# MiloszKrajewski/K4os.Compression.LZ4

Hardware: AMD Instinct MI355X
Metric: GiB/s encode+decode on batched 64 KiB blocks; bit-exact vs C# ref (higher is better)
Workload: dtype u8

## Files before the change

experiments/parse_cost_order/fit.py:

```python
import ctypes as C, os, sys, subprocess, numpy as np
ROOT = os.path.dirname(os.path.dirname(os.path.dirname(os.path.abspath(__file__))))
sys.path.insert(0, ROOT)
WORK = sys.argv[1]
from k4os.compression.lz4_amd import corpus
so = os.path.join(WORK, "libstudy.so")
lib = C.CDLL(so)
n, bs = 4096, 65536
cache = os.path.join(WORK, "blocks.npy")
if os.path.exists(cache): blocks = np.load(cache)
else:
    blocks = corpus.silesia_like_blocks(n, bs, seed=2); np.save(cache, blocks)
uidx = np.array([ci + 12 * t for ci in range(12) for t in range(32)])
ub = np.ascontiguousarray(blocks[uidx])
off = (np.arange(384, dtype=np.uint64) * bs); lens = np.full(384, bs, np.int32)
def stats(o, l):
    out = np.zeros((384, 8), np.uint32)
    lib.study_stats(ub.ctypes.data_as(C.POINTER(C.c_uint8)), C.c_void_p(off.ctypes.data), C.c_void_p(lens.ctypes.data), C.c_longlong(384), C.c_uint32(o), C.c_uint32(l), C.c_void_p(out.ctypes.data), C.c_int(8), C.c_uint32(0))
    return out[:, :6].astype(np.float64), out[:, 6].astype(np.float64)
b = np.arange(n); u = (b % 12) * 32 + (b // 12) % 32
ls = np.zeros(384); ln = np.zeros(384); ms = np.zeros(384); mn = np.zeros(384)
for f in ("parent_blocks", "oracleP_blocks", "oracleQ_blocks"):
    res = np.load(os.path.join(WORK, "%s.npy" % f))
    for r in res:
        d = (r[:, 1] - r[:, 0]) / 1e5; k = r[:, 2].astype(int)
        np.add.at(ls, u[k == 4], d[k == 4]); np.add.at(ln, u[k == 4], 1)
        np.add.at(ms, u[k != 4], d[k != 4]); np.add.at(mn, u[k != 4], 1)
lds = np.where(ln > 0, ls / np.maximum(ln, 1), np.nan); mem = np.where(mn > 0, ms / np.maximum(mn, 1), np.nan)
both = (ln >= 2) & (mn >= 2)
ratio = np.median(mem[both] / lds[both]); print("ratio", ratio, "both", both.sum(), "lds known", (ln > 0).sum())
truth = np.where(np.isnan(lds), mem / ratio, lds)
np.save(os.path.join(WORK, "truth.npy"), truth)
names = corpus.SILESIA_NAMES
def evaluate(tag, est):
    e = est[u] + 1e-9 * np.random.default_rng(0).random(n)
    t = truth[u]
    cut = np.sort(e)[::-1][2303]
    inl = e >= cut
    tail_mem = (t[~inl] * ratio).max(); tail_lds = t[inl].max()
    tcut = np.sort(t)[::-1][2303]
    mis = ((t >= tcut) & ~inl).sum()
# ... 28 lines not shown
```

experiments/parse_cost_order/fit_stats.cpp:

```cpp
#include "hip/hip_runtime.h"
#include "k4lz4_decode.hpp"
#include "k4lz4_encode_fast.hpp"
#include "k4lz4_parse.hpp"
#include <vector>

namespace k4 {
__global__ void stats_kernel(BatchArgs a, uint32_t off, uint32_t len, uint32_t *out, uint32_t cap = 0)
{
    __shared__ __attribute__((aligned(16))) uint32_t lds[PCOST_WAVES_PER_WG][4096 + PARSE_SEEN_DWORDS];
    const int lane = lane_id();
    const uint32_t wave = uni(threadIdx.x >> 6);
    const long long b = (long long)blockIdx.x * PCOST_WAVES_PER_WG + (long long)wave;
    if (b >= a.n) return;
    const uint32_t src_len = (uint32_t)a.srcLen[b];
    uint32_t o = off, s = len;
    if (o + s > src_len) { o = 0; s = s < src_len ? s : src_len; }
    ParseStats st; st.max_rounds = cap;
    const uint32_t nseq = parse_block<1, false, true>(a.src + a.srcOff[b] + o, s, nullptr, (uint16_t *)lds[wave], lds[wave] + 4096, lane, nullptr, &st);
    if (lane == 0) { uint32_t *w = out + 8 * b; w[0] = st.rounds; w[1] = st.slow; w[2] = nseq; w[3] = st.groups; w[4] = st.lazies; w[5] = st.longs; w[6] = st.covered; }
}
}

extern "C" int study_stats(const uint8_t *src, const uint64_t *srcOff, const int32_t *srcLen, long long n, uint32_t off, uint32_t len, uint32_t *out, int threads, uint32_t cap)
{
    k4::BatchArgs a{};
    a.src = src; a.srcOff = srcOff; a.srcLen = srcLen; a.n = n; a.accel = 1;
    k4emu::launch_fn(dim3((unsigned)((n + k4::PCOST_WAVES_PER_WG - 1) / k4::PCOST_WAVES_PER_WG)), dim3(64 * k4::PCOST_WAVES_PER_WG), [=] { k4::stats_kernel(a, off, len, out, cap); }, threads);
    return 0;
}
```

k4os/compression/lz4_amd/csrc/k4lz4_capi.hip:

```cpp
#include <hip/hip_runtime.h>
#include <stdint.h>
#include <stdio.h>
#include <stdlib.h>
#include <string.h>
#include <algorithm>
#include <atomic>
#include <memory>
#include <new>
#include <condition_variable>
#include <functional>
#include <map>
#include <mutex>
#include <string>
#include <thread>
#include <chrono>
#include <vector>

#include "../../../../include/k4lz4.h"
#include "k4lz4_decode.hpp"
#include "k4lz4_encode_fast.hpp"
#include "k4lz4_parse.hpp"
#include "k4lz4_pickle.hpp"
#include "k4lz4_segments.hpp"
#include "k4lz4_encode_hc.hpp"
// ... 554 lines not shown
            a.seg_first = sg.first; a.seg_items = sg.items; a.seg_snaps = sg.snaps;
            seg = true;
        }
        auto segments_start = [&]() -> int {
            if (!seg) return K4LZ4_OK;
            K4_HIP(ctx, hipEventRecord(ctx->ev_fork, stream));
            K4_HIP(ctx, hipStreamWaitEvent(ctx->aux2, ctx->ev_fork, 0));
            hipLaunchKernelGGL(k4::k4_encode_seg_kernel, dim3((unsigned)((sg.max_items + k4::ENCODE_WAVES_PER_WG - 1) / k4::ENCODE_WAVES_PER_WG)), dim3(64 * k4::ENCODE_WAVES_PER_WG), 0, ctx->aux2, a, sg);
            K4_HIP(ctx, hipEventRecord(ctx->ev_join2, ctx->aux2));
            return K4LZ4_OK;
        };
        auto segments_join = [&]() -> int {
            if (!seg) return K4LZ4_OK;
            K4_HIP(ctx, hipStreamWaitEvent(stream, ctx->ev_join2, 0));
            hipLaunchKernelGGL(k4::k4_seg_join_kernel, dim3((unsigned)std::min<int64_t>(k4::SEG_MAX_BLOCKS, cnt)), dim3(64), 0, stream, a, sg);
            return K4LZ4_OK;
        };
        if (dd && dd->dict) {
            a.dict = dd->dict; a.dictOff = dd->off + first; a.dictLen = dd->len + first;
            a.dictMode = dd->mode ? dd->mode + first : nullptr;
        }
        if (reorder && parse_path && kind == KIND_ENCODE && ctx->parse_pcost) {
            const int64_t wgs = std::min<int64_t>((cnt + k4::PARSE_MAX_WAVES - 1) / k4::PARSE_MAX_WAVES, ctx->cu_count);
            const size_t need = (size_t)wgs * (k4::PARSE_MAX_WAVES - k4::PARSE_LDS_TABLES) * 16384;
            if (need > ctx->d_parse_cap) K4_HIP(ctx, hipStreamSynchronize(stream));
            const int rcp = grow(ctx, &ctx->d_parse, &ctx->d_parse_cap, need, false);
            if (rcp != K4LZ4_OK) return rcp;
            a.cost = d_cost; a.hist = d_hist; a.order_out = d_order;
            K4_HIP(ctx, hipMemsetAsync(d_hist, 0, 2 * k4::PCOST_BUCKETS * 4, stream));
            k4::ParseCost pc = ctx->pcost_fit;
            pc.tables = (uint32_t *)ctx->d_parse;
            hipLaunchKernelGGL(static_cast<void (*)(k4::BatchArgs, k4::ParseCost)>(k4::k4_cost_kernel), dim3((unsigned)wgs), dim3(64 * k4::PARSE_MAX_WAVES), 0, stream, a, pc);
            hipLaunchKernelGGL(k4::k4_order_kernel, dim3((unsigned)((cnt + 255) / 256)), dim3(256), 0, stream, a, 0xffffffffu, 1);
            a.order = d_order;
        }
        else if (reorder) {
            a.cost = d_cost; a.hist = d_hist; a.order_out = d_order;
            K4_HIP(ctx, hipMemsetAsync(d_hist, 0, (2 * k4::COST_BUCKETS + 16) * 4, stream));
            hipLaunchKernelGGL(k4::k4_cost_kernel, dim3((unsigned)cnt), dim3(64), 0, stream, a, encode_like ? 0 : 1,
                               kind == KIND_ENCODE && parse_path ? k4::COST_SAMPLE_PARSE : k4::COST_SAMPLE);
            const bool two_kernels = kind == KIND_ENCODE && !a.prof && cnt > 512 && !(flags & K4LZ4_FLAG_NO_SPLIT) &&
                                     cnt > 8 * (int64_t)ctx->cu_count && ctx->split_pct <= 0;
            k4::BatchArgs ao = a;
            ao.first = two_kernels ? (uint32_t)ctx->cost_pct : 0u;
            ao.total = (uint32_t)((int64_t)ctx->lds_floor_per_cu * (int64_t)ctx->cu_count);
            hipLaunchKernelGGL(k4::k4_order_kernel, dim3((unsigned)((cnt + 255) / 256)), dim3(256), 0, stream, ao, (uint32_t)lds_share(ctx, cnt));
            a.order = d_order;
            if (two_kernels) a.split = d_hist + 2 * k4::COST_BUCKETS;
        }
        const unsigned wg4 = (unsigned)((cnt + k4::DECODE_WAVES_PER_WG - 1) / k4::DECODE_WAVES_PER_WG);
        bool parse_here = kind == KIND_ENCODE && (parse_path || (parse_seg_path && (a.order || cnt == 1)));
        const bool big_ok = ctx->parse_big && ctx->parse_inline_emit;
        bool any_small = true, any_big = big_ok;
        if (parse_here && hostLen) {
            any_small = false; any_big = false;
            for (int64_t i = 0; i < cnt && !(any_small && (any_big || !big_ok)); i++) {
                const int32_t len = hostLen[first + i];
                if (len >= (int32_t)k4::PARSE_MIN_LEN && len < k4::LIMIT_64K) any_small = true;
                else if (len >= k4::LIMIT_64K && big_ok) any_big = true;
            }
            parse_here = any_small || any_big;
        }
        int64_t waves = 0, nwg = 0, nwg_seg = 0;
        const bool seg_two_step = seg && parse_here && parse_seg_path;
        bool queue = false, slot_recs = false;
        size_t o_meta = 0, o_gtab = 0;
        if (parse_here) {
            waves = std::max<int64_t>(1, std::min<int64_t>(ctx->parse_waves, (cnt + ctx->cu_count - 1) / ctx->cu_count));
            queue = (ctx->parse_queue || parse_persistent || parse_seg_path) && a.order && cnt > waves * (int64_t)ctx->cu_count;
// ... 1387 lines not shown
    dict_layout(dv, w, fam, nt, nd, (size_t)n, nslots);
    const size_t up_bytes = (size_t)((uint8_t *)w.cost - (uint8_t *)w.toff);
    if (list) {
        try { sc.host.assign(up_bytes, 0); } catch (...) { return fail(ctx, K4LZ4_E_NOMEM, "out of host memory"); }
        auto host = [&](auto *p) { return (decltype(p))(sc.host.data() + ((uint8_t *)p - (uint8_t *)w.toff)); };
        dict_words(*list, host(w.toff), host(w.tlen), host(w.eoff), host(w.elen), host(w.etab));
        sc.table = list->table; sc.kept = list->keptLen;
    } else {
        sc.table.clear(); sc.kept.clear();
    }
    K4_HIP(ctx, order_after_ctx(ctx, stream));
    if (list) {
        K4_HIP(ctx, hipMemcpyAsync(w.toff, sc.host.data(), up_bytes, hipMemcpyHostToDevice, stream));
        K4_HIP(ctx, hipEventRecord(sc.ev, stream));
    }
    K4_HIP(ctx, hipMemsetAsync(w.head, 0, DICT_HEAD_WORDS * 4, stream));
    if (list) fam.load(stream, (unsigned)nt, dict, w.toff, w.tlen, w.tables);
    if (n > 0) {
        if (fam.slots) K4_HIP(ctx, hipMemsetAsync(w.slots, 0, nslots * fam.table_bytes, stream));
        k4::BatchArgs o{};
        o.srcLen = b.srcLen; o.n = n; o.cost = w.cost; o.hist = w.head + 64; o.order_out = w.order;
        const unsigned g256 = (unsigned)((n + 255) / 256);
        hipLaunchKernelGGL(k4::k4_dict_cost_kernel, dim3(g256), dim3(256), 0, stream, o);
        hipLaunchKernelGGL(k4::k4_order_kernel, dim3(g256), dim3(256), 0, stream, o, 0xffffffffu);
        const k4lz4_dict_set::Family *f = list ? nullptr : &(set->*fam.in_set);
        const DictTables t = list ? DictTables{dict, w.eoff, w.elen, w.etab, w.tables, (int)nd}
                                  : DictTables{set->buf, f->eoff, f->elen, f->etab, f->tables, (int)set->nDict};
        fam.encode(stream, (unsigned)wgs, b, t, w, ctx->d_status, level);
    }
    rc = hipGetLastError() != hipSuccess ? fail(ctx, K4LZ4_E_HIP, std::string(who) + ": kernel launch failed") : K4LZ4_OK;
    mark_busy(ctx, stream);
    return rc;
}

int dict_encode_device(k4lz4_ctx *ctx, const DictFamily &fam, int level, int flags, const DictBatch &b, const DictSource &s, void *stream)
{
    int rc = dict_encode_args(ctx, fam, level, flags, b, s);
    if (rc != K4LZ4_OK) return rc;
    DictList l;
    if (!s.of_set && (rc = dict_list(ctx, fam.min_kept, fam.who, s.dictOff, s.dictLen, s.nDict, nullptr, l)) != K4LZ4_OK) return rc;
    K4_HIP(ctx, hipSetDevice(ctx->device));
    return dict_encode_run(ctx, fam, level, b, s.dict, s.of_set ? nullptr : &l, s.set, (hipStream_t)stream);
}

int dict_encode_host(k4lz4_ctx *ctx, const DictFamily &fam, int level, int flags, const DictBatch &b, const DictSource &s)
{
    int rc = dict_encode_args(ctx, fam, level, flags, b, s);
// ... 338 lines not shown
    ctx->hc_cand_lds = getenv("K4LZ4_HC_CAND_MEM") == nullptr;
    if (const char *e = getenv("K4LZ4_HC_CAND_DYNLDS")) ctx->hc_cand_dynlds = std::max(0, std::min(65536, atoi(e)));
    if (const char *e = getenv("K4LZ4_HC_SEGS")) { const int v = atoi(e); ctx->hc_segs = v >= 4 ? 4 : (v >= 2 ? 2 : (v == 1 ? 1 : 0)); }
    if (const char *e = getenv("K4LZ4_HC_MEM_PCT")) ctx->hc_mem_pct = std::max(0, std::min(100, atoi(e)));
    ctx->use_segments = getenv("K4LZ4_NO_SEGMENTS") == nullptr;
    if (const char *e = getenv("K4LZ4_SEG_MIN")) ctx->seg_min = (uint32_t)std::max(65536 + 4096, atoi(e));
    if (const char *e = getenv("K4LZ4_SEG_TARGET")) ctx->seg_target = ctx->seg_target_max = (uint32_t)std::max(8192, atoi(e));
    if (const char *e = getenv("K4LZ4_SEG_TARGET_MAX")) ctx->seg_target_max = (uint32_t)std::max(8192, atoi(e));
    if (const char *e = getenv("K4LZ4_SEG_WARM")) ctx->seg_warm = (uint32_t)std::max(0, atoi(e));
    if (const char *e = getenv("K4LZ4_SEG_SPIN_MAX")) ctx->seg_spin_max = (uint32_t)std::max(0, atoi(e));
    if (const char *e = getenv("K4LZ4_SEG_DIV")) ctx->seg_div = (uint32_t)std::max(0, atoi(e));
    if (const char *e = getenv("K4LZ4_PICKLE_SPLIT_MIN")) ctx->pickle_split_min = std::max(0, atoi(e));
    if (const char *e = getenv("K4LZ4_STAGE_THREADS")) ctx->stage_threads = std::max(0, std::min(63, atoi(e) - 1));
    ctx->use_parse = getenv("K4LZ4_NO_PARSE") == nullptr;
    ctx->parse_queue = getenv("K4LZ4_PARSE_QUEUE") != nullptr;
    ctx->parse_persist = getenv("K4LZ4_NO_PERSIST") == nullptr;
    ctx->parse_big = getenv("K4LZ4_NO_PARSE_BIG") == nullptr;
    ctx->parse_seg = getenv("K4LZ4_NO_PARSE_SEG") == nullptr;
    ctx->hc_records = getenv("K4LZ4_NO_HC_RECORDS") == nullptr;
    ctx->parse_pcost = getenv("K4LZ4_NO_PCOST") == nullptr || getenv("K4LZ4_PCOST") != nullptr;
    if (const char *e = getenv("K4LZ4_PCOST_FIT")) {
        unsigned v[9];
        if (sscanf(e, "%u,%u,%u,%u,%u,%u,%u,%u,%u", &v[0], &v[1], &v[2], &v[3], &v[4], &v[5], &v[6], &v[7], &v[8]) == 9 && v[0] >= k4::PARSE_MIN_LEN && v[0] < 65536u)
            ctx->pcost_fit = k4::ParseCost{v[0], v[1], v[2], v[3], v[4], v[5], v[6], v[7], v[8], nullptr};
    }
    ctx->parse_migrate = getenv("K4LZ4_NO_MIGRATE") == nullptr;
    ctx->parse_inline_emit = getenv("K4LZ4_NO_INLINE_EMIT") == nullptr;
    if (const char *e = getenv("K4LZ4_PARSE_WAVES")) ctx->parse_waves = std::max(1, std::min(k4::PARSE_MAX_WAVES, atoi(e)));
    ctx->trace = getenv("K4LZ4_TRACE") != nullptr;
    if (e != hipSuccess) { delete ctx; return hip_fail(nullptr, e, "hipStreamCreate"); }
    *out = ctx;
    return K4LZ4_OK;
}

void k4lz4_ctx_destroy(k4lz4_ctx *ctx)
{
    if (!ctx) return;
    (void)hipSetDevice(ctx->device);
    if (ctx->stream) { (void)hipStreamSynchronize(ctx->stream); (void)hipStreamDestroy(ctx->stream); }
    if (ctx->aux) { (void)hipStreamSynchronize(ctx->aux); (void)hipStreamDestroy(ctx->aux); }
    if (ctx->aux2) { (void)hipStreamSynchronize(ctx->aux2); (void)hipStreamDestroy(ctx->aux2); }
    if (ctx->ev_join2) (void)hipEventDestroy(ctx->ev_join2);
    if (ctx->d_seg) (void)hipFree(ctx->d_seg);
    if (ctx->d_seg_first) (void)hipFree(ctx->d_seg_first);
    if (ctx->ev_fork) (void)hipEventDestroy(ctx->ev_fork);
    if (ctx->ev_join) (void)hipEventDestroy(ctx->ev_join);
    if (ctx->ev_busy) (void)hipEventDestroy(ctx->ev_busy);
// ... 2447 lines not shown
```

k4os/compression/lz4_amd/csrc/k4lz4_encode_fast.hpp:

```cpp
#pragma once
#include "k4lz4_common.hpp"

namespace k4 {

#ifndef K4_SEG_WAVES_MIN
#define K4_SEG_WAVES_MIN 5
#endif
#ifndef K4_GTAB_DUTY
#define K4_GTAB_DUTY 3
#endif
#ifndef K4_PACE
#define K4_PACE 1
#endif

template <int TYPE> struct FastTable;

template <> struct FastTable<1> {
    uint16_t *t;
    __device__ __forceinline__ static uint32_t hash(const uint8_t *p) { return (ld32u(p) * 2654435761u) >> (32 - 13); }
    __device__ __forceinline__ static uint32_t hash_of(uint32_t seq, uint32_t) { return (seq * 2654435761u) >> (32 - 13); }
    __device__ __forceinline__ uint32_t get(uint32_t h) const { return t[h]; }
    __device__ __forceinline__ void put(uint32_t h, uint32_t pos) const { t[h] = (uint16_t)pos; }
    __device__ __forceinline__ uint32_t get_nt(uint32_t h) const
    {
#ifndef K4_HOST_EMU
        return __builtin_nontemporal_load(t + h);
#else
        return t[h];
#endif
    }
    __device__ __forceinline__ void put_nt(uint32_t h, uint32_t pos) const
    {
#ifndef K4_HOST_EMU
        __builtin_nontemporal_store((uint16_t)pos, t + h);
#else
        t[h] = (uint16_t)pos;
#endif
    }
};
template <> struct FastTable<0> {
    uint32_t *t;
    __device__ __forceinline__ static uint32_t hash(const uint8_t *p)
    {
        return (uint32_t)(((ld64u(p) << 24) * 889523592379ull) >> (64 - 12));
    }
    __device__ __forceinline__ static uint32_t hash_of(uint32_t seq, uint32_t n0)
    {
        return (uint32_t)((((((uint64_t)n0) << 32) | seq) << 24) * 889523592379ull >> (64 - 12));
    }
    __device__ __forceinline__ uint32_t get(uint32_t h) const { return t[h]; }
    __device__ __forceinline__ void put(uint32_t h, uint32_t pos) const { t[h] = pos; }
};
template <> struct FastTable<2> {
    uint32_t *t;
    __device__ __forceinline__ static uint32_t hash(const uint8_t *p) { return (ld32u(p) * 2654435761u) >> (32 - 12); }
    __device__ __forceinline__ static uint32_t hash_of(uint32_t seq, uint32_t) { return (seq * 2654435761u) >> (32 - 12); }
    __device__ __forceinline__ uint32_t get(uint32_t h) const { return t[h]; }
    __device__ __forceinline__ void put(uint32_t h, uint32_t pos) const { t[h] = pos; }
};

__device__ __forceinline__ uint32_t probe_offset(uint32_t j, uint32_t accel)
{
    if (j == 0) return 0;
    const uint32_t M = accel * 64u - 2u + j;
    const uint32_t q = M >> 6;
    return 1u + 32u * q * (q - 1u) + q * (M - 64u * q + 1u) - 32u * accel * (accel - 1u);
}

__device__ __forceinline__ uint32_t wave_count(const uint8_t *a, const uint8_t *b, uint32_t maxn, int lane)
{
    uint32_t done = 0;
    for (;;) {
        const uint32_t i = done + 4u * (uint32_t)lane;
        uint32_t neq = 0;
        if (i < maxn) {
            const uint32_t x = ld32u(a + i) ^ ld32u(b + i);
            const uint32_t avail = maxn - i < 4u ? maxn - i : 4u;
            const uint32_t e = x ? (uint32_t)(__ffs(x) - 1) >> 3 : 4u;
            neq = e < avail ? e : avail;
        }
        const unsigned long long notfull = ballot(neq != 4u);
// ... 763 lines not shown
    const uint32_t l = bkt >> 1;
    return ((bkt & 1u) ? 7ull : 5ull) << (l - 1u);
}

template <int NB>
__device__ __forceinline__ void suffix_counts(const uint32_t *hist, uint32_t *before, uint32_t *above)
{
    static_assert(NB % 64 == 0 && NB <= 4096, "whole waves of counts; their totals fit one wave");
    const uint32_t lane = (uint32_t)lane_id(), wave = uni(threadIdx.x >> 6), waves = blockDim.x >> 6;
    for (uint32_t c = wave; c < (uint32_t)NB / 64u; c += waves) {
        const uint32_t k = (uint32_t)NB - 1u - (64u * c + lane);
        const uint32_t v = hist[k], incl = wave_inclusive_scan(v);
        before[k] = incl - v;
        if (lane == 63u) above[c] = incl;
    }
    __syncthreads();
    if (wave == 0u) {
        const uint32_t v = lane < (uint32_t)NB / 64u ? above[lane] : 0u, incl = wave_inclusive_scan(v);
        if (lane < (uint32_t)NB / 64u) above[lane] = incl - v;
    }
    __syncthreads();
}

template <int NB>
__device__ __forceinline__ void order_by_bucket(const BatchArgs &a)
{
    __shared__ uint32_t before[NB], above[NB / 64];
    suffix_counts<NB>(a.hist, before, above);
    const long long b = (long long)blockIdx.x * 256 + threadIdx.x;
    if (b >= a.n) return;
    const uint32_t bkt = a.cost[b];
    const uint32_t pos = before[bkt] + above[((uint32_t)NB - 1u - bkt) >> 6] + atomicAdd(&a.hist[NB + bkt], 1u);
    a.order_out[pos] = (uint32_t)b;
}

__global__ __launch_bounds__(256) void k4_order_kernel(BatchArgs a, uint32_t lds_max = 0xffffffffu, int fine = 0)
{
    if (fine) { order_by_bucket<COST_BUCKETS_FINE>(a); return; }
    if (blockIdx.x == 0 && threadIdx.x == 0 && a.first != 0u) {
        unsigned long long all = 0;
        for (uint32_t k = 0; k < (uint32_t)COST_BUCKETS; k++) all += (unsigned long long)a.hist[k] * bucket_cost(k);
        const unsigned long long want = all / 100ull * (unsigned long long)a.first;
        unsigned long long have = 0, cnt = 0;
        for (int k = COST_BUCKETS - 1; k >= 0 && have < want; k--) {
            const unsigned long long c = a.hist[k], w = bucket_cost((uint32_t)k);
            if (have + c * w <= want) { have += c * w; cnt += c; }
            else { const unsigned long long part = (want - have + w - 1ull) / w; cnt += part; have = want; }
        }
        const unsigned long long floor_n = (unsigned long long)a.total < (unsigned long long)a.n ? (unsigned long long)a.total : (unsigned long long)a.n;
        if (cnt < floor_n) cnt = floor_n;
        if (cnt > (unsigned long long)a.n) cnt = (unsigned long long)a.n;
        if (cnt > (unsigned long long)lds_max) cnt = (unsigned long long)lds_max;
        a.hist[2 * COST_BUCKETS] = (uint32_t)cnt;
    }
    order_by_bucket<COST_BUCKETS>(a);
}
// ... 133 lines not shown
```

k4os/compression/lz4_amd/csrc/k4lz4_parse.hpp:

```cpp
#pragma once
#include "k4lz4_encode_fast.hpp"
#include <type_traits>
#ifdef K4_PARSE_DEBUG
#include <stdio.h>
#include <stdlib.h>
#endif

namespace k4 {

#ifndef K4_PARSE_K
#define K4_PARSE_K 1
#endif

constexpr uint32_t PARSE_REC_STRIDE = 16448u;
static_assert(PARSE_REC_STRIDE >= ((uint32_t)LIMIT_64K - 1u - 6u) / 4u + 1u + 62u, "a block below LIMIT_64K has at most (LIMIT_64K - 1 - 6) / 4 sequences; a round adds at most 64 / 4 + 1");
constexpr uint32_t PARSE_MIN_LEN = 128u;
constexpr uint32_t PARSE_REST = 0xffffffffu;
constexpr uint32_t PARSE_BIG = 0xfffffffeu;
constexpr int PARSE_MAX_WAVES = 16;
constexpr int PARSE_LDS_TABLES = 9;
constexpr int PARSE_SEEN_DWORDS = 128;

constexpr int PARSE_LDS_DWORDS = 4096 * PARSE_LDS_TABLES + PARSE_SEEN_DWORDS * PARSE_MAX_WAVES + 4;

// ... 65 lines not shown
constexpr uint32_t HOP_LONG = 0x100u, HOP_LAZY = 0x200u, HOP_END = 0x400u, HOP_INVALID = 0x800u, HOP_TABMISS = 0x1000u;

struct ParseStats { uint32_t rounds, slow, groups, lazies, longs; uint32_t covered, max_rounds; };
constexpr int PARSE_FLUSH = -2;

struct ParseCtl {
    uint32_t *free_slots;
    uint32_t rec_cap;
    int claimed;
    bool resume;
    uint32_t c, sbase, sj, nrec, long_seen, long_rounds;
    bool test, more;
    uint32_t cut_pos;
    bool dry, stopped;
};

template <int K, bool GT, bool DRY = false, int TT = 1, bool SEG = false>
__device__ __forceinline__ uint32_t parse_block(const uint8_t *src, const uint32_t U, uint2 *recs, void *tabv, uint32_t *seen, const int lane, unsigned long long *pc = nullptr,
                                                ParseStats *stats = nullptr, ParseCtl *ctl = nullptr, SegRun *sr = nullptr)
{
    static_assert(!SEG || (TT != 1 && K == 1 && !DRY), "segments: byU32 blocks, one sub-window per round");
    typedef FastTable<TT> Table;
    static_assert(TT == 1 || K == 1, "byU32 tables: one sub-window per round");
    constexpr bool U32 = TT != 1;
    Table tab;
    tab.t = (decltype(tab.t))tabv;
    constexpr uint32_t SEEN_SHIFT = TT == 1 ? 1u : 0u;
    ParseStats st = {0u, 0u, 0u, 0u, 0u, U, DRY && stats ? uni(stats->max_rounds) : 0u};
#define K4_ST(field, v) do { if (DRY) st.field += (v); } while (0)
#ifdef K4_PARSE_PROF
    unsigned long long pt[8] = {0, 0, 0, 0, 0, 0, 0, 0}, pn[8] = {0, 0, 0, 0, 0, 0, 0, 0}, plast = 0;
    const unsigned long long pbegin = prof_now<true>();
#define K4_PT(i) do { const unsigned long long t_ = prof_now<true>(); pt[i] += t_ - plast; plast = t_; } while (0)
#define K4_PN(i, v) (pn[i] += (v))
#define K4_TIC() const unsigned long long tic_ = (unsigned long long)__builtin_readcyclecounter()
#define K4_TOC(i) (pt[i] += (unsigned long long)__builtin_readcyclecounter() - tic_)
#else
#define K4_TIC() ((void)0)
#define K4_TOC(i) ((void)0)
#define K4_PT(i) ((void)0)
#define K4_PN(i, v) ((void)0)
#endif
#if defined(K4_PARSE_PROF) && !defined(K4_PARSE_PROF_SPLIT)
#define K4_TICA() K4_TIC()
#define K4_TOCA(i) K4_TOC(i)
#else
#define K4_TICA() ((void)0)
#define K4_TOCA(i) ((void)0)
#endif
#if defined(K4_PARSE_PROF) && defined(K4_PARSE_PROF_SPLIT)
#define K4_TICB() const unsigned long long ticb_ = (unsigned long long)__builtin_readcyclecounter()
#define K4_TOCB(i) (pt[i] += (unsigned long long)__builtin_readcyclecounter() - ticb_)
#define K4_TICC() const unsigned long long ticc_ = (unsigned long long)__builtin_readcyclecounter()
#define K4_TOCC(i) (pt[i] += (unsigned long long)__builtin_readcyclecounter() - ticc_)
#else
#define K4_TICB() ((void)0)
#define K4_TOCB(i) ((void)0)
#define K4_TICC() ((void)0)
#define K4_TOCC(i) ((void)0)
#endif
    const uint32_t mfl1 = U - (uint32_t)MFLIMIT + 1u;
    const uint32_t matchlimit = U - (uint32_t)LASTLITERALS;
    const unsigned long long me = 1ull << lane, below_me = me - 1ull;

    const bool resumed = ctl && ctl->resume;
    if (!resumed) for (int k = lane; k < 1024; k += 64) ((uint4 *)tabv)[k] = make_uint4(0u, 0u, 0u, 0u);
    for (int k = lane; k < PARSE_SEEN_DWORDS; k += 64) seen[k] = 0u;
    wave_sync();

    uint32_t cut_pos = 0xffffffffu;
    bool dry = false, cut_hit = false;
    uint32_t seg_begin = 0u;
    if (SEG) {
        const uint32_t ef = uni(sr->emit_from), sa = uni(sr->stop_at);
        seg_begin = uni(sr->begin);
        dry = ef != 0u;
        cut_pos = ef ? ef : sa;
    }
    if (SEG && !resumed && seg_begin != 0u) {
        if (lane == 0) tab.put(Table::hash(src + seg_begin), seg_begin);
        wave_sync();
    }
    uint32_t c = seg_begin + 1u;
    uint32_t sbase = seg_begin + 1u;
    bool test = false;
    uint32_t sj = 0u;
    uint32_t nrec = 0u;

    uint32_t seq[K], n0[K], n1[K], n2[K];
// ... 852 lines not shown
        if (!p.queue) return;
    }
}


__global__ __launch_bounds__(64 * PARSE_MAX_WAVES) void k4_parse_kernel(BatchArgs a, ParseArgs p)
{
    __shared__ __attribute__((aligned(16))) uint32_t lds[PARSE_LDS_DWORDS];
    parse_kernel_body<K4_PARSE_K>(a, p, lds);
}

__global__ __launch_bounds__(64 * PARSE_MAX_WAVES) void k4_parse_big_kernel(BatchArgs a, ParseArgs p)
{
    __shared__ __attribute__((aligned(16))) uint32_t lds[PARSE_LDS_DWORDS];
    if (a.flags & FLAG_X32) parse_kernel_body<1, 2>(a, p, lds);
    else parse_kernel_body<1, 0>(a, p, lds);
}


struct ParseCost {
    uint32_t sample, max_rounds;
    uint32_t round, slow, seq, group, lazy, lng;
    uint32_t base;
    uint32_t *tables;
};
constexpr ParseCost PCOST_FIT = {2048u, 10u, 999u, 0u, 104u, 0u, 18u, 181u, 835300u, nullptr};
constexpr int PCOST_BUCKETS = COST_BUCKETS_FINE;
constexpr int PCOST_WAVES_PER_WG = PARSE_MAX_WAVES;

__device__ __forceinline__ uint32_t pcost_bucket(unsigned long long cost)
{
    if (cost < 16384ull) return 0u;
    const uint32_t l = 63u - (uint32_t)__clzll((long long)cost);
    const uint32_t b = 32u * (l - 14u) + (uint32_t)((cost >> (l - 5u)) & 31ull) + 1u;
    return b < (uint32_t)PCOST_BUCKETS ? b : (uint32_t)PCOST_BUCKETS - 1u;
}

__device__ __forceinline__ void parse_cost_body(const BatchArgs &a, const ParseCost &pc, uint32_t *lds, uint32_t *far)
{
    const int lane = lane_id();
    const uint32_t wave = uni(threadIdx.x >> 6);
    uint32_t *seen = lds + 4096u * (uint32_t)PARSE_LDS_TABLES + (uint32_t)PARSE_SEEN_DWORDS * wave;
    for (long long b = (long long)blockIdx.x * PARSE_MAX_WAVES + (long long)wave; b < a.n; b += (long long)gridDim.x * PARSE_MAX_WAVES) {
        const int src_len = a.srcLen[b];
        unsigned long long cost = 0ull;
        if (src_len >= (int)PARSE_MIN_LEN && src_len < LIMIT_64K) {
            const uint32_t sample = (uint32_t)src_len < pc.sample ? (uint32_t)src_len : pc.sample;
            const uint8_t *src = a.src + a.srcOff[b];
            ParseStats st;
            st.max_rounds = pc.max_rounds;
            uint32_t nseq;
            if (wave < (uint32_t)PARSE_LDS_TABLES) nseq = parse_block<1, false, true>(src, sample, nullptr, lds + 4096u * wave, seen, lane, nullptr, &st);
            else nseq = parse_block<1, true, true>(src, sample, nullptr, far + 4096u * (wave - (uint32_t)PARSE_LDS_TABLES), seen, lane, nullptr, &st);
            const unsigned long long ns = (unsigned long long)pc.round * st.rounds + (unsigned long long)pc.slow * st.slow + (unsigned long long)pc.seq * nseq +
                                          (unsigned long long)pc.group * st.groups + (unsigned long long)pc.lazy * st.lazies + (unsigned long long)pc.lng * st.longs;
            cost = ns * (unsigned long long)(uint32_t)src_len / (st.covered ? st.covered : 1u) + (((unsigned long long)pc.base * (unsigned long long)(uint32_t)src_len) >> 16);
        } else if (src_len > 0) {
            cost = 40ull * (unsigned long long)(uint32_t)src_len;
        }
        if (lane == 0) {
            const uint32_t bkt = pcost_bucket(cost);
            a.cost[b] = bkt;
            atomicAdd(&a.hist[bkt], 1u);
        }
    }
}

__global__ __launch_bounds__(64 * PARSE_MAX_WAVES) void k4_cost_kernel(BatchArgs a, ParseCost pc)
{
    __shared__ __attribute__((aligned(16))) uint32_t lds[4096 * PARSE_LDS_TABLES + PARSE_SEEN_DWORDS * PARSE_MAX_WAVES];
    parse_cost_body(a, pc, lds, pc.tables + 4096ull * (unsigned long long)(PARSE_MAX_WAVES - PARSE_LDS_TABLES) * (unsigned long long)blockIdx.x);
}

#ifdef K4_HOST_EMU
inline void k4_pcost_kernel(BatchArgs a)
{
    __shared__ __attribute__((aligned(16))) uint32_t lds[4096 * PARSE_LDS_TABLES + PARSE_SEEN_DWORDS * PARSE_MAX_WAVES];
    __shared__ __attribute__((aligned(16))) uint32_t far[4096 * (PARSE_MAX_WAVES - PARSE_LDS_TABLES)];
    parse_cost_body(a, PCOST_FIT, lds, far);
}
inline void k4_porder_kernel(BatchArgs a) { k4_order_kernel(a, 0xffffffffu, 1); }
#endif


constexpr int EMIT_WAVES_PER_WG = 4;

template <bool HC, bool BIG>
__device__ __forceinline__ bool emit_records(const uint8_t *src, const uint32_t U, uint8_t *dst, const int dst_cap, const uint2 *recs, const uint32_t nseq, const int lane, EmitState &st)
{
    const bool limited = dst_cap < compress_bound((int)U);
    const uint64_t olimit = (uint64_t)(dst_cap < 0 ? 0 : dst_cap);
    uint32_t op = st.op, emitted_to = st.emitted_to;
    uint2 rn = make_uint2(0u, 0u);
    if ((uint32_t)lane < nseq) rn = rec_load(recs + lane);
    for (uint32_t base = 0u; base < nseq; base += 64u) {
        const uint32_t n = nseq - base < 64u ? nseq - base : 64u;
        const bool mine = (uint32_t)lane < n;
        const uint2 r = rn;
        if (base + 64u + (uint32_t)lane < nseq) rn = rec_load(recs + base + 64u + (uint32_t)lane);
        const uint32_t pos = r.x, cpos = r.x - (r.y & 0xffffu);
        uint32_t code = r.y >> 16;
        if (BIG) {
// ... 153 lines not shown
```

Before: 62.43.

## Use small LDS-only sample hash tables for parse cost and deterministic order kernel

The parse-cost pre-pass now dry-runs each block's sample with a smaller 12-bit uint16 hash table. All sixteen waves' tables then fit in LDS, so the global 'far' scratch buffer, its growth and synchronisation are removed. The cost weights are refit for the new table. The order kernel is rewritten to assign positions by prefix counting within capped workgroups rather than global atomics, making the ordering deterministic. It also shrinks the histogram memset, at the cost of rescanning preceding cost entries per workgroup and possibly less accurate cost estimates from the smaller hash.

Result: faster. 63.96, median of 6 (+2.4%).

```diff
diff --git a/experiments/parse_cost_order/fit.py b/experiments/parse_cost_order/fit.py
--- a/experiments/parse_cost_order/fit.py
+++ b/experiments/parse_cost_order/fit.py
@@ -15,7 +15,7 @@
 off = (np.arange(384, dtype=np.uint64) * bs); lens = np.full(384, bs, np.int32)
 def stats(o, l):
     out = np.zeros((384, 8), np.uint32)
-    lib.study_stats(ub.ctypes.data_as(C.POINTER(C.c_uint8)), C.c_void_p(off.ctypes.data), C.c_void_p(lens.ctypes.data), C.c_longlong(384), C.c_uint32(o), C.c_uint32(l), C.c_void_p(out.ctypes.data), C.c_int(8), C.c_uint32(0))
+    lib.study_stats(ub.ctypes.data_as(C.POINTER(C.c_uint8)), C.c_void_p(off.ctypes.data), C.c_void_p(lens.ctypes.data), C.c_longlong(384), C.c_uint32(o), C.c_uint32(l), C.c_void_p(out.ctypes.data), C.c_int(8), C.c_uint32(0), C.c_int(0))
     return out[:, :6].astype(np.float64), out[:, 6].astype(np.float64)
 b = np.arange(n); u = (b % 12) * 32 + (b // 12) % 32
 ls = np.zeros(384); ln = np.zeros(384); ms = np.zeros(384); mn = np.zeros(384)
diff --git a/experiments/parse_cost_order/fit_sample_table.py b/experiments/parse_cost_order/fit_sample_table.py
--- /dev/null
+++ b/experiments/parse_cost_order/fit_sample_table.py
@@ -0,0 +1,52 @@
+import ctypes as C, os, sys, numpy as np
+from scipy.optimize import nnls
+from scipy.stats import spearmanr
+ROOT = os.path.dirname(os.path.dirname(os.path.dirname(os.path.abspath(__file__))))
+sys.path.insert(0, ROOT)
+from k4os.compression.lz4_amd import corpus
+WORK = sys.argv[1]
+n, bs = 4096, 65536
+cache = os.path.join(WORK, "blocks.npy")
+if os.path.exists(cache): blocks = np.load(cache)
+else:
+    blocks = corpus.silesia_like_blocks(n, bs, seed=2); np.save(cache, blocks)
+uidx = np.array([ci + 12 * t for ci in range(12) for t in range(32)])
+ub = np.ascontiguousarray(blocks[uidx])
+off = (np.arange(384, dtype=np.uint64) * bs); lens = np.full(384, bs, np.int32)
+names = corpus.SILESIA_NAMES
+b = np.arange(n); u = (b % 12) * 32 + (b // 12) % 32
+
+
+def stats(lib, o, l, cap, form):
+    out = np.zeros((384, 8), np.uint32)
+    lib.study_stats(ub.ctypes.data_as(C.POINTER(C.c_uint8)), C.c_void_p(off.ctypes.data), C.c_void_p(lens.ctypes.data), C.c_longlong(384), C.c_uint32(o), C.c_uint32(l),
+                    C.c_void_p(out.ctypes.data), C.c_int(8), C.c_uint32(cap), C.c_int(form))
+    return out[:, :6].astype(np.float64), out[:, 6].astype(np.float64)
+
+
+libs = {bits: C.CDLL(os.path.join(WORK, "libstudy%d.so" % bits)) for bits in (13, 12, 11)}
+tp = os.path.join(WORK, "truth.npy")
+if os.path.exists(tp):
+    truth = np.load(tp); print("truth: stamped LDS durations (truth.npy)")
+else:
+    full, _ = stats(libs[13], 0, bs, 0, 0)
+    truth = full @ np.array([1.28e-3, 0.84e-3, 0.094e-3, 0.036e-3, 0.0, 0.70e-3]) + 0.23
+    print("truth: the whole block's counts by section 2's weights (no stamps here)")
+for ci, nm in enumerate(names):
+    print("  %-8s truth ms mean %.3f min %.3f max %.3f" % (nm, truth[ci * 32:(ci + 1) * 32].mean(), truth[ci * 32:(ci + 1) * 32].min(), truth[ci * 32:(ci + 1) * 32].max()))
+t_all = truth[u]
+tcut = np.sort(t_all)[::-1][2303]
+for bits in (13, 12, 11):
+    for (l, cap) in ((2048, 10), (2048, 12), (1024, 12), (2048, 14), (1024, 14), (1024, 16), (1536, 12), (768, 12)):
+        s, cov = stats(libs[bits], 0, l, cap, 0 if bits == 13 else 1)
+        sc = s * (bs / np.maximum(cov, 1))[:, None]
+        A = np.c_[sc, np.ones(384)]
+        w, _ = nnls(A, truth)
+        est = A @ w
+        e = est[u] + 1e-9 * np.random.default_rng(0).random(n)
+        inl = e >= np.sort(e)[::-1][2303]
+        mis = int(((t_all >= tcut) & ~inl).sum())
+        share = {nm: float(inl[np.arange(ci, n, 12)].mean()) for ci, nm in enumerate(names) if nm in ("nci", "xml", "samba", "mozilla", "mr", "ooffice", "osdb", "sao")}
+        fit = ",".join(str(int(round(x * 1e6))) for x in w)
+        print("bits %2d sample %4d limit %2d: rho %.3f misplaced %4d heaviest without LDS %.3f ms | K4LZ4_PCOST_FIT=%d,%d,%s | LDS share %s" % (
+            bits, l, cap, spearmanr(est, truth).correlation, mis, t_all[~inl].max(), l, cap, fit, " ".join("%s %.2f" % kv for kv in share.items())))
diff --git a/experiments/parse_cost_order/fit_stats.cpp b/experiments/parse_cost_order/fit_stats.cpp
--- a/experiments/parse_cost_order/fit_stats.cpp
+++ b/experiments/parse_cost_order/fit_stats.cpp
@@ -5,7 +5,7 @@
 #include <vector>
 
 namespace k4 {
-__global__ void stats_kernel(BatchArgs a, uint32_t off, uint32_t len, uint32_t *out, uint32_t cap = 0)
+__global__ void stats_kernel(BatchArgs a, uint32_t off, uint32_t len, uint32_t *out, uint32_t cap = 0, int form = 0)
 {
     __shared__ __attribute__((aligned(16))) uint32_t lds[PCOST_WAVES_PER_WG][4096 + PARSE_SEEN_DWORDS];
     const int lane = lane_id();
@@ -16,15 +16,17 @@
     uint32_t o = off, s = len;
     if (o + s > src_len) { o = 0; s = s < src_len ? s : src_len; }
     ParseStats st; st.max_rounds = cap;
-    const uint32_t nseq = parse_block<1, false, true>(a.src + a.srcOff[b] + o, s, nullptr, (uint16_t *)lds[wave], lds[wave] + 4096, lane, nullptr, &st);
+    uint32_t nseq;
+    if (form == 0) nseq = parse_block<1, false, true>(a.src + a.srcOff[b] + o, s, nullptr, (uint16_t *)lds[wave], lds[wave] + 4096, lane, nullptr, &st);
+    else nseq = parse_block<1, false, true, 3>(a.src + a.srcOff[b] + o, s, nullptr, (uint16_t *)lds[wave], lds[wave] + 4096, lane, nullptr, &st);
     if (lane == 0) { uint32_t *w = out + 8 * b; w[0] = st.rounds; w[1] = st.slow; w[2] = nseq; w[3] = st.groups; w[4] = st.lazies; w[5] = st.longs; w[6] = st.covered; }
 }
 }
 
-extern "C" int study_stats(const uint8_t *src, const uint64_t *srcOff, const int32_t *srcLen, long long n, uint32_t off, uint32_t len, uint32_t *out, int threads, uint32_t cap)
+extern "C" int study_stats(const uint8_t *src, const uint64_t *srcOff, const int32_t *srcLen, long long n, uint32_t off, uint32_t len, uint32_t *out, int threads, uint32_t cap, int form)
 {
     k4::BatchArgs a{};
     a.src = src; a.srcOff = srcOff; a.srcLen = srcLen; a.n = n; a.accel = 1;
-    k4emu::launch_fn(dim3((unsigned)((n + k4::PCOST_WAVES_PER_WG - 1) / k4::PCOST_WAVES_PER_WG)), dim3(64 * k4::PCOST_WAVES_PER_WG), [=] { k4::stats_kernel(a, off, len, out, cap); }, threads);
+    k4emu::launch_fn(dim3((unsigned)((n + k4::PCOST_WAVES_PER_WG - 1) / k4::PCOST_WAVES_PER_WG)), dim3(64 * k4::PCOST_WAVES_PER_WG), [=] { k4::stats_kernel(a, off, len, out, cap, form); }, threads);
     return 0;
 }
diff --git a/k4os/compression/lz4_amd/csrc/k4lz4_capi.hip b/k4os/compression/lz4_amd/csrc/k4lz4_capi.hip
--- a/k4os/compression/lz4_amd/csrc/k4lz4_capi.hip
+++ b/k4os/compression/lz4_amd/csrc/k4lz4_capi.hip
@@ -600,16 +600,10 @@
         }
         if (reorder && parse_path && kind == KIND_ENCODE && ctx->parse_pcost) {
             const int64_t wgs = std::min<int64_t>((cnt + k4::PARSE_MAX_WAVES - 1) / k4::PARSE_MAX_WAVES, ctx->cu_count);
-            const size_t need = (size_t)wgs * (k4::PARSE_MAX_WAVES - k4::PARSE_LDS_TABLES) * 16384;
-            if (need > ctx->d_parse_cap) K4_HIP(ctx, hipStreamSynchronize(stream));
-            const int rcp = grow(ctx, &ctx->d_parse, &ctx->d_parse_cap, need, false);
-            if (rcp != K4LZ4_OK) return rcp;
             a.cost = d_cost; a.hist = d_hist; a.order_out = d_order;
-            K4_HIP(ctx, hipMemsetAsync(d_hist, 0, 2 * k4::PCOST_BUCKETS * 4, stream));
-            k4::ParseCost pc = ctx->pcost_fit;
-            pc.tables = (uint32_t *)ctx->d_parse;
-            hipLaunchKernelGGL(static_cast<void (*)(k4::BatchArgs, k4::ParseCost)>(k4::k4_cost_kernel), dim3((unsigned)wgs), dim3(64 * k4::PARSE_MAX_WAVES), 0, stream, a, pc);
-            hipLaunchKernelGGL(k4::k4_order_kernel, dim3((unsigned)((cnt + 255) / 256)), dim3(256), 0, stream, a, 0xffffffffu, 1);
+            K4_HIP(ctx, hipMemsetAsync(d_hist, 0, k4::PCOST_BUCKETS * 4, stream));
+            hipLaunchKernelGGL(static_cast<void (*)(k4::BatchArgs, k4::ParseCost)>(k4::k4_cost_kernel), dim3((unsigned)wgs), dim3(64 * k4::PARSE_MAX_WAVES), 0, stream, a, ctx->pcost_fit);
+            hipLaunchKernelGGL(k4::k4_order_kernel, dim3(k4::order_workgroups(cnt)), dim3(256), 0, stream, a, 0xffffffffu, 1);
             a.order = d_order;
         }
         else if (reorder) {
@@ -622,7 +616,7 @@
             k4::BatchArgs ao = a;
             ao.first = two_kernels ? (uint32_t)ctx->cost_pct : 0u;
             ao.total = (uint32_t)((int64_t)ctx->lds_floor_per_cu * (int64_t)ctx->cu_count);
-            hipLaunchKernelGGL(k4::k4_order_kernel, dim3((unsigned)((cnt + 255) / 256)), dim3(256), 0, stream, ao, (uint32_t)lds_share(ctx, cnt));
+            hipLaunchKernelGGL(k4::k4_order_kernel, dim3(k4::order_workgroups(cnt)), dim3(256), 0, stream, ao, (uint32_t)lds_share(ctx, cnt));
             a.order = d_order;
             if (two_kernels) a.split = d_hist + 2 * k4::COST_BUCKETS;
         }
@@ -2056,7 +2050,7 @@
         o.srcLen = b.srcLen; o.n = n; o.cost = w.cost; o.hist = w.head + 64; o.order_out = w.order;
         const unsigned g256 = (unsigned)((n + 255) / 256);
         hipLaunchKernelGGL(k4::k4_dict_cost_kernel, dim3(g256), dim3(256), 0, stream, o);
-        hipLaunchKernelGGL(k4::k4_order_kernel, dim3(g256), dim3(256), 0, stream, o, 0xffffffffu);
+        hipLaunchKernelGGL(k4::k4_order_kernel, dim3(k4::order_workgroups(n)), dim3(256), 0, stream, o, 0xffffffffu);
         const k4lz4_dict_set::Family *f = list ? nullptr : &(set->*fam.in_set);
         const DictTables t = list ? DictTables{dict, w.eoff, w.elen, w.etab, w.tables, (int)nd}
                                   : DictTables{set->buf, f->eoff, f->elen, f->etab, f->tables, (int)set->nDict};
@@ -2441,7 +2435,7 @@
     if (const char *e = getenv("K4LZ4_PCOST_FIT")) {
         unsigned v[9];
         if (sscanf(e, "%u,%u,%u,%u,%u,%u,%u,%u,%u", &v[0], &v[1], &v[2], &v[3], &v[4], &v[5], &v[6], &v[7], &v[8]) == 9 && v[0] >= k4::PARSE_MIN_LEN && v[0] < 65536u)
-            ctx->pcost_fit = k4::ParseCost{v[0], v[1], v[2], v[3], v[4], v[5], v[6], v[7], v[8], nullptr};
+            ctx->pcost_fit = k4::ParseCost{v[0], v[1], v[2], v[3], v[4], v[5], v[6], v[7], v[8]};
     }
     ctx->parse_migrate = getenv("K4LZ4_NO_MIGRATE") == nullptr;
     ctx->parse_inline_emit = getenv("K4LZ4_NO_INLINE_EMIT") == nullptr;
diff --git a/k4os/compression/lz4_amd/csrc/k4lz4_encode_fast.hpp b/k4os/compression/lz4_amd/csrc/k4lz4_encode_fast.hpp
--- a/k4os/compression/lz4_amd/csrc/k4lz4_encode_fast.hpp
+++ b/k4os/compression/lz4_amd/csrc/k4lz4_encode_fast.hpp
@@ -17,6 +17,7 @@
 
 template <> struct FastTable<1> {
     uint16_t *t;
+    static constexpr int ZERO_UINT4 = 1024;
     __device__ __forceinline__ static uint32_t hash(const uint8_t *p) { return (ld32u(p) * 2654435761u) >> (32 - 13); }
     __device__ __forceinline__ static uint32_t hash_of(uint32_t seq, uint32_t) { return (seq * 2654435761u) >> (32 - 13); }
     __device__ __forceinline__ uint32_t get(uint32_t h) const { return t[h]; }
@@ -40,6 +41,7 @@
 };
 template <> struct FastTable<0> {
     uint32_t *t;
+    static constexpr int ZERO_UINT4 = 1024;
     __device__ __forceinline__ static uint32_t hash(const uint8_t *p)
     {
         return (uint32_t)(((ld64u(p) << 24) * 889523592379ull) >> (64 - 12));
@@ -53,10 +55,22 @@
 };
 template <> struct FastTable<2> {
     uint32_t *t;
+    static constexpr int ZERO_UINT4 = 1024;
     __device__ __forceinline__ static uint32_t hash(const uint8_t *p) { return (ld32u(p) * 2654435761u) >> (32 - 12); }
     __device__ __forceinline__ static uint32_t hash_of(uint32_t seq, uint32_t) { return (seq * 2654435761u) >> (32 - 12); }
     __device__ __forceinline__ uint32_t get(uint32_t h) const { return t[h]; }
     __device__ __forceinline__ void put(uint32_t h, uint32_t pos) const { t[h] = pos; }
+};
+#ifndef K4_SAMPLE_HASH_BITS
+#define K4_SAMPLE_HASH_BITS 12
+#endif
+template <> struct FastTable<3> {
+    static constexpr int ZERO_UINT4 = (2 << K4_SAMPLE_HASH_BITS) / 16;
+    uint16_t *t;
+    __device__ __forceinline__ static uint32_t hash(const uint8_t *p) { return (ld32u(p) * 2654435761u) >> (32 - K4_SAMPLE_HASH_BITS); }
+    __device__ __forceinline__ static uint32_t hash_of(uint32_t seq, uint32_t) { return (seq * 2654435761u) >> (32 - K4_SAMPLE_HASH_BITS); }
+    __device__ __forceinline__ uint32_t get(uint32_t h) const { return t[h]; }
+    __device__ __forceinline__ void put(uint32_t h, uint32_t pos) const { t[h] = (uint16_t)pos; }
 };
 
 __device__ __forceinline__ uint32_t probe_offset(uint32_t j, uint32_t accel)
@@ -866,16 +880,64 @@
     __syncthreads();
 }
 
+constexpr int ORDER_MAX_WGS = 256;
+inline unsigned order_workgroups(long long n)
+{
+    long long g = (n + 255) / 256;
+    if (g > ORDER_MAX_WGS) g = ORDER_MAX_WGS;
+    const long long bound = n > 0 ? (1ll << 24) / n : ORDER_MAX_WGS;
+    if (g > bound) g = bound < 16 ? 16 : bound;
+    return (unsigned)(g < 1 ? 1 : g);
+}
+constexpr int ORDER_COPIES = 8;
 template <int NB>
 __device__ __forceinline__ void order_by_bucket(const BatchArgs &a)
 {
     __shared__ uint32_t before[NB], above[NB / 64];
+    __shared__ uint32_t base[ORDER_COPIES][NB], wcnt[4][NB];
+    const uint32_t tid = threadIdx.x, lane = (uint32_t)lane_id(), wave = uni(threadIdx.x >> 6);
+    for (uint32_t k = tid; k < (uint32_t)(ORDER_COPIES * NB); k += 256u) (&base[0][0])[k] = 0u;
+    for (uint32_t k = tid; k < (uint32_t)(4 * NB); k += 256u) (&wcnt[0][0])[k] = 0u;
     suffix_counts<NB>(a.hist, before, above);
-    const long long b = (long long)blockIdx.x * 256 + threadIdx.x;
-    if (b >= a.n) return;
-    const uint32_t bkt = a.cost[b];
-    const uint32_t pos = before[bkt] + above[((uint32_t)NB - 1u - bkt) >> 6] + atomicAdd(&a.hist[NB + bkt], 1u);
-    a.order_out[pos] = (uint32_t)b;
+    const long long per = (((long long)a.n + (long long)gridDim.x - 1) / (long long)gridDim.x + 255) & ~255ll;
+    if ((long long)blockIdx.x * per >= (long long)a.n) return;
+    const long long lo = (long long)blockIdx.x * per, hi = lo + per < (long long)a.n ? lo + per : (long long)a.n;
+    for (long long i = (long long)tid; i < lo; i += 256) {
+        const uint32_t bkt = a.cost[i];
+        atomicAdd(&base[lane & (uint32_t)(ORDER_COPIES - 1)][bkt < (uint32_t)NB ? bkt : (uint32_t)NB - 1u], 1u);
+    }
+    __syncthreads();
+    for (uint32_t k = tid; k < (uint32_t)NB; k += 256u) {
+        uint32_t s = before[k] + above[((uint32_t)NB - 1u - k) >> 6];
+        for (int c = 0; c < ORDER_COPIES; c++) s += base[c][k];
+        base[0][k] = s;
+    }
+    __syncthreads();
+    for (long long i0 = lo; i0 < hi; i0 += 256) {
+        const long long b = i0 + (long long)tid;
+        const bool have = b < hi;
+        uint32_t bkt = 0xffffffffu;
+        if (have) { bkt = a.cost[b]; if (bkt >= (uint32_t)NB) bkt = (uint32_t)NB - 1u; }
+        uint32_t rank = 0u, cnt = 0u;
+        unsigned long long todo = ballot(have);
+        while (todo) {
+            const uint32_t v = readlane_u32(bkt, ctz64(todo));
+            const unsigned long long m = ballot(bkt == v);
+            if (bkt == v) { rank = (uint32_t)__popcll(m & ((1ull << lane) - 1ull)); cnt = (uint32_t)__popcll(m); }
+            todo &= ~m;
+        }
+        const bool leader = have && rank == 0u;
+        if (leader) wcnt[wave][bkt] = cnt;
+        __syncthreads();
+        if (have) {
+            uint32_t pos = base[0][bkt] + rank;
+            for (uint32_t w = 0; w < wave; w++) pos += wcnt[w][bkt];
+            if ((long long)pos < (long long)a.n) a.order_out[pos] = (uint32_t)b;
+        }
+        __syncthreads();
+        if (leader) { atomicAdd(&base[0][bkt], cnt); wcnt[wave][bkt] = 0u; }
+        __syncthreads();
+    }
 }
 
 __global__ __launch_bounds__(256) void k4_order_kernel(BatchArgs a, uint32_t lds_max = 0xffffffffu, int fine = 0)
diff --git a/k4os/compression/lz4_amd/csrc/k4lz4_parse.hpp b/k4os/compression/lz4_amd/csrc/k4lz4_parse.hpp
--- a/k4os/compression/lz4_amd/csrc/k4lz4_parse.hpp
+++ b/k4os/compression/lz4_amd/csrc/k4lz4_parse.hpp
@@ -111,10 +111,12 @@
     static_assert(!SEG || (TT != 1 && K == 1 && !DRY), "segments: byU32 blocks, one sub-window per round");
     typedef FastTable<TT> Table;
     static_assert(TT == 1 || K == 1, "byU32 tables: one sub-window per round");
-    constexpr bool U32 = TT != 1;
+    static_assert(TT != 3 || (DRY && !GT && K == 1), "the sample's table: dry runs in LDS only");
+    constexpr bool U32 = TT == 0 || TT == 2;
     Table tab;
     tab.t = (decltype(tab.t))tabv;
     constexpr uint32_t SEEN_SHIFT = TT == 1 ? 1u : 0u;
+    static_assert(TT != 3 || (1 << K4_SAMPLE_HASH_BITS) <= 32 * PARSE_SEEN_DWORDS, "one bit of `seen` per hash value of the sample's table");
     ParseStats st = {0u, 0u, 0u, 0u, 0u, U, DRY && stats ? uni(stats->max_rounds) : 0u};
 #define K4_ST(field, v) do { if (DRY) st.field += (v); } while (0)
 #ifdef K4_PARSE_PROF
@@ -153,7 +155,7 @@
     const unsigned long long me = 1ull << lane, below_me = me - 1ull;
 
     const bool resumed = ctl && ctl->resume;
-    if (!resumed) for (int k = lane; k < 1024; k += 64) ((uint4 *)tabv)[k] = make_uint4(0u, 0u, 0u, 0u);
+    if (!resumed) for (int k = lane; k < Table::ZERO_UINT4; k += 64) ((uint4 *)tabv)[k] = make_uint4(0u, 0u, 0u, 0u);
     for (int k = lane; k < PARSE_SEEN_DWORDS; k += 64) seen[k] = 0u;
     wave_sync();
 
@@ -1052,11 +1054,13 @@
     uint32_t sample, max_rounds;
     uint32_t round, slow, seq, group, lazy, lng;
     uint32_t base;
-    uint32_t *tables;
 };
-constexpr ParseCost PCOST_FIT = {2048u, 10u, 999u, 0u, 104u, 0u, 18u, 181u, 835300u, nullptr};
+constexpr ParseCost PCOST_FIT = {2048u, 12u, 1166u, 0u, 85u, 0u, 42u, 131u, 739622u};
 constexpr int PCOST_BUCKETS = COST_BUCKETS_FINE;
 constexpr int PCOST_WAVES_PER_WG = PARSE_MAX_WAVES;
+constexpr int PCOST_TABLE_DWORDS = FastTable<3>::ZERO_UINT4 * 4;
+constexpr int PCOST_LDS_DWORDS = (PCOST_TABLE_DWORDS + PARSE_SEEN_DWORDS) * PCOST_WAVES_PER_WG;
+static_assert(PCOST_LDS_DWORDS * 4 <= 160 * 1024, "sixteen sample tables and their `seen` sets in one CU's LDS");
 
 __device__ __forceinline__ uint32_t pcost_bucket(unsigned long long cost)
 {
@@ -1066,11 +1070,11 @@
     return b < (uint32_t)PCOST_BUCKETS ? b : (uint32_t)PCOST_BUCKETS - 1u;
 }
 
-__device__ __forceinline__ void parse_cost_body(const BatchArgs &a, const ParseCost &pc, uint32_t *lds, uint32_t *far)
+__device__ __forceinline__ void parse_cost_body(const BatchArgs &a, const ParseCost &pc, uint32_t *lds)
 {
     const int lane = lane_id();
     const uint32_t wave = uni(threadIdx.x >> 6);
-    uint32_t *seen = lds + 4096u * (uint32_t)PARSE_LDS_TABLES + (uint32_t)PARSE_SEEN_DWORDS * wave;
+    uint32_t *seen = lds + (uint32_t)PCOST_TABLE_DWORDS * (uint32_t)PCOST_WAVES_PER_WG + (uint32_t)PARSE_SEEN_DWORDS * wave;
     for (long long b = (long long)blockIdx.x * PARSE_MAX_WAVES + (long long)wave; b < a.n; b += (long long)gridDim.x * PARSE_MAX_WAVES) {
         const int src_len = a.srcLen[b];
         unsigned long long cost = 0ull;
@@ -1079,9 +1083,7 @@
             const uint8_t *src = a.src + a.srcOff[b];
             ParseStats st;
             st.max_rounds = pc.max_rounds;
-            uint32_t nseq;
-            if (wave < (uint32_t)PARSE_LDS_TABLES) nseq = parse_block<1, false, true>(src, sample, nullptr, lds + 4096u * wave, seen, lane, nullptr, &st);
-            else nseq = parse_block<1, true, true>(src, sample, nullptr, far + 4096u * (wave - (uint32_t)PARSE_LDS_TABLES), seen, lane, nullptr, &st);
+            const uint32_t nseq = parse_block<1, false, true, 3>(src, sample, nullptr, lds + (uint32_t)PCOST_TABLE_DWORDS * wave, seen, lane, nullptr, &st);
             const unsigned long long ns = (unsigned long long)pc.round * st.rounds + (unsigned long long)pc.slow * st.slow + (unsigned long long)pc.seq * nseq +
                                           (unsigned long long)pc.group * st.groups + (unsigned long long)pc.lazy * st.lazies + (unsigned long long)pc.lng * st.longs;
             cost = ns * (unsigned long long)(uint32_t)src_len / (st.covered ? st.covered : 1u) + (((unsigned long long)pc.base * (unsigned long long)(uint32_t)src_len) >> 16);
@@ -1098,16 +1100,15 @@
 
 __global__ __launch_bounds__(64 * PARSE_MAX_WAVES) void k4_cost_kernel(BatchArgs a, ParseCost pc)
 {
-    __shared__ __attribute__((aligned(16))) uint32_t lds[4096 * PARSE_LDS_TABLES + PARSE_SEEN_DWORDS * PARSE_MAX_WAVES];
-    parse_cost_body(a, pc, lds, pc.tables + 4096ull * (unsigned long long)(PARSE_MAX_WAVES - PARSE_LDS_TABLES) * (unsigned long long)blockIdx.x);
+    __shared__ __attribute__((aligned(16))) uint32_t lds[PCOST_LDS_DWORDS];
+    parse_cost_body(a, pc, lds);
 }
 
 #ifdef K4_HOST_EMU
 inline void k4_pcost_kernel(BatchArgs a)
 {
-    __shared__ __attribute__((aligned(16))) uint32_t lds[4096 * PARSE_LDS_TABLES + PARSE_SEEN_DWORDS * PARSE_MAX_WAVES];
-    __shared__ __attribute__((aligned(16))) uint32_t far[4096 * (PARSE_MAX_WAVES - PARSE_LDS_TABLES)];
-    parse_cost_body(a, PCOST_FIT, lds, far);
+    __shared__ __attribute__((aligned(16))) uint32_t lds[PCOST_LDS_DWORDS];
+    parse_cost_body(a, PCOST_FIT, lds);
 }
 inline void k4_porder_kernel(BatchArgs a) { k4_order_kernel(a, 0xffffffffu, 1); }
 #endif
```
